# vobbilis/kubernetes-rca-system

Measured on AMD Instinct MI355X. Metric: pod·timesteps scored/s + end-to-end RCA top-k latency (ms), 1M-pod mesh, higher is better.
Workload: dtype f32 (f64 window sums, int64 fixed-point ranks)

## Files before the change

kubernetes-rca-system_amd/csrc/score.hip:

```cpp
#include "krca_common.h"

#pragma clang fp contract(off)

namespace {

constexpr double kVarEps = 1e-12;

__global__ __launch_bounds__(256) void usage_flags_kernel(const float2* __restrict__ usage, int64_t P,
                                                          uint8_t* __restrict__ flags) {
  const int64_t stride = (int64_t)gridDim.x * blockDim.x;
  for (int64_t p = (int64_t)blockIdx.x * blockDim.x + threadIdx.x; p < P; p += stride) {
    const float2 u = usage[p];
    flags[p] = (u.x > 80.f ? KRCA_F_CPU80 : 0u) | (u.x > 90.f ? KRCA_F_CPU90 : 0u) |
               (u.y > 80.f ? KRCA_F_MEM80 : 0u) | (u.y > 90.f ? KRCA_F_MEM90 : 0u);
  }
}

struct StepState {
  double s1, s2;
  int cnt;
  double al, bl;
};

__device__ __forceinline__ void step(StepState& st, float v, float old, double Wd, double epsB, double thr2,
                                     bool last) {
  const double vd = (double)v;
  const double od = (double)old;
  const double A = fma(Wd, vd, -st.s1);
  const double B = fma(Wd, st.s2, -(st.s1 * st.s1));
  st.cnt += (B > epsB) && (fma(A, A, -(thr2 * B)) > 0.0);
  if (last) {
    st.al = A;
    st.bl = B;
  }
  st.s1 = (st.s1 + vd) - od;
  st.s2 = fma(-od, od, fma(vd, vd, st.s2));
}

struct NoEpisodes {
  static constexpr bool kTrack = false;
  struct Args {};
  __device__ __forceinline__ explicit NoEpisodes(Args) {}
};

struct TimelineOut {
  int32_t* onset;
  int32_t* last;
  int32_t* count;
  float* peak;
  int8_t* lead;
  uint8_t* n_metrics;
};

template <class Ep>
__device__ __forceinline__ void step(StepState& st, float v, float old, double Wd, double epsB, double thr2,
                                     bool last, Ep& ep, int t) {
  if constexpr (!Ep::kTrack) {
    step(st, v, old, Wd, epsB, thr2, last);
  } else {
    const double vd = (double)v;
    const double od = (double)old;
    const double A = fma(Wd, vd, -st.s1);
    const double B = fma(Wd, st.s2, -(st.s1 * st.s1));
    const bool exceed = (B > epsB) && (fma(A, A, -(thr2 * B)) > 0.0);
    st.cnt += exceed;
    if (exceed) ep.hit(t, A, B);
    if (last) {
      st.al = A;
      st.bl = B;
    }
    st.s1 = (st.s1 + vd) - od;
    st.s2 = fma(-od, od, fma(vd, vd, st.s2));
  }
}

struct Episodes {
  static constexpr bool kTrack = true;
  struct Args {
    int gap, min_count;
    TimelineOut out;
  };
  int gap, min_count;
  int c_on, c_last, c_cnt;
  float c_peak;
  int k_on, k_last, k_cnt;
  float k_peak;
  __device__ __forceinline__ explicit Episodes(const Args& a)
      : gap(a.gap), min_count(a.min_count), c_on(-1), c_last(-1), c_cnt(0), c_peak(0.f), k_on(-1), k_last(-1),
        k_cnt(0), k_peak(-1.f) {}
  __device__ __forceinline__ void close() {
    if (c_cnt >= min_count && c_peak >= k_peak) {
      k_on = c_on;
      k_last = c_last;
      k_cnt = c_cnt;
      k_peak = c_peak;
    }
  }
  __device__ __forceinline__ void hit(int t, double A, double B) {
    const float z = (float)(fabs(A) / sqrt(B));
    if (c_cnt > 0 && t - c_last <= gap) {
      c_last = t;
      ++c_cnt;
      c_peak = fmaxf(c_peak, z);
    } else {
      close();
      c_on = c_last = t;
      c_cnt = 1;
      c_peak = z;
    }
  }
};

struct StreamEpisodes : Episodes {
  struct Args {
    int gap, min_count, H;
    int32_t* state;
    TimelineOut out;
  };
  int H;
  bool c_dirty, k_dirty;
  __device__ __forceinline__ explicit StreamEpisodes(const Args& a)
      : Episodes(Episodes::Args{a.gap, a.min_count, a.out}), H(a.H), c_dirty(false), k_dirty(false) {}
  __device__ __forceinline__ void load(const int32_t* p, int64_t S, int64_t sl) {
    c_on = p[sl];
    c_last = p[S + sl];
    c_cnt = p[2 * S + sl];
    c_peak = __builtin_bit_cast(float, p[3 * S + sl]);
    k_on = p[4 * S + sl];
    k_last = p[5 * S + sl];
    k_cnt = p[6 * S + sl];
    k_peak = __builtin_bit_cast(float, p[7 * S + sl]);
  }
  __device__ __forceinline__ void store(int32_t* p, int64_t S, int64_t sl) const {
    if (c_dirty) {
      p[sl] = c_on;
      p[S + sl] = c_last;
      p[2 * S + sl] = c_cnt;
      p[3 * S + sl] = __builtin_bit_cast(int32_t, c_peak);
    }
    if (k_dirty) {
      p[4 * S + sl] = k_on;
      p[5 * S + sl] = k_last;
      p[6 * S + sl] = k_cnt;
      p[7 * S + sl] = __builtin_bit_cast(int32_t, k_peak);
    }
  }
  __device__ __forceinline__ void close(int now) {
    if (c_cnt >= min_count && (k_cnt == 0 || now - k_last >= H || c_peak >= k_peak)) {
      k_on = c_on;
      k_last = c_last;
      k_cnt = c_cnt;
      k_peak = c_peak;
      k_dirty = true;
    }
  }
  __device__ __forceinline__ void hit(int t, double A, double B) {
    const float z = (float)(fabs(A) / sqrt(B));
    c_dirty = true;
    if (c_cnt > 0 && t - c_last <= gap) {
      c_last = t;
      ++c_cnt;
      c_peak = fmaxf(c_peak, z);
    } else {
      close(t);
      c_on = c_last = t;
      c_cnt = 1;
      c_peak = z;
    }
  }
};

__device__ __forceinline__ void timeline_combine(bool has, int e_on, int e_last, int e_cnt, float e_peak, int gap,
                                                 int64_t s, bool active, int M, const TimelineOut& o) {
  const int lane = threadIdx.x & 63;
  const int m = lane & (M - 1);
  float ap = has ? e_peak : -1.f;
  int am = m;
  for (int off = 1; off < M; off <<= 1) {
    const float op = __shfl_xor(ap, off, 64);
    const int om = __shfl_xor(am, off, 64);
    if (op > ap || (op == ap && om < am)) {
      ap = op;
      am = om;
    }
  }
  const int src = (lane & ~(M - 1)) + am;
  const int64_t a_on = __shfl(e_on, src, 64), a_last = __shfl(e_last, src, 64);
  const bool mem = has && (int64_t)e_on <= a_last + gap && a_on <= (int64_t)e_last + gap;
  long long first = mem ? (((long long)e_on << 8) | m) : INT64_MAX;
  int lastv = mem ? e_last : -1;
  int cnt = mem ? e_cnt : 0;
  int nm = mem ? 1 : 0;
  for (int off = 1; off < M; off <<= 1) {
    const long long of = __shfl_xor(first, off, 64);
    first = of < first ? of : first;
    const int ol = __shfl_xor(lastv, off, 64);
    lastv = ol > lastv ? ol : lastv;
    cnt += __shfl_xor(cnt, off, 64);
    nm += __shfl_xor(nm, off, 64);
  }
  if (!active || m != 0) return;
  const int64_t p = s / M;
  o.onset[p] = nm ? (int32_t)(first >> 8) : -1;
  o.last[p] = lastv;
  o.count[p] = cnt;
  o.peak[p] = nm ? ap : 0.f;
  o.lead[p] = nm ? (int8_t)(first & 0xff) : (int8_t)-1;
  o.n_metrics[p] = (uint8_t)nm;
}

__device__ __forceinline__ void timeline_epilogue(Episodes& ep, int64_t s, bool active, int M,
                                                  const TimelineOut& o) {
  ep.close();
  timeline_combine(active && ep.k_cnt > 0, ep.k_on, ep.k_last, ep.k_cnt, ep.k_peak, ep.gap, s, active, M, o);
}

__device__ __forceinline__ void stream_timeline_epilogue(const StreamEpisodes& ep, int now, int64_t s, bool active,
                                                         int M, const TimelineOut& o) {
  const bool k_ok = ep.k_cnt > 0 && now - ep.k_last < ep.H;
  const bool c_ok = ep.c_cnt >= ep.min_count && now - ep.c_last < ep.H;
  const bool use_c = c_ok && (!k_ok || ep.c_peak >= ep.k_peak);
  timeline_combine(active && (use_c || k_ok), use_c ? ep.c_on : ep.k_on, use_c ? ep.c_last : ep.k_last,
                   use_c ? ep.c_cnt : ep.k_cnt, use_c ? ep.c_peak : ep.k_peak, ep.gap, s, active, M, o);
}

__device__ __forceinline__ void pod_epilogue(const StepState& st, double epsB, int64_t s, bool active, int M, int T,
                                             const float* __restrict__ xs, int64_t S,
                                             float* __restrict__ z_last, float* __restrict__ score,
                                             int32_t* __restrict__ n_exceed, uint8_t* __restrict__ flags) {
  const bool has_z = st.bl > epsB;
  const float z = has_z ? (float)(st.al / sqrt(st.bl)) : 0.f;
  const int m = (int)(s & (M - 1));
  float vlast = (active && T > 0) ? xs[(int64_t)(T - 1) * S] : 0.f;
  unsigned f = 0;
  if (m == 0) f = (vlast > 80.f ? KRCA_F_CPU80 : 0u) | (vlast > 90.f ? KRCA_F_CPU90 : 0u);
  if (m == 1) f = (vlast > 80.f ? KRCA_F_MEM80 : 0u) | (vlast > 90.f ? KRCA_F_MEM90 : 0u);
  float az = fabsf(z);
  int cnt = st.cnt;
  for (int off = 1; off < M; off <<= 1) {
    az = fmaxf(az, __shfl_xor(az, off, 64));
    cnt += __shfl_xor(cnt, off, 64);
    f |= __shfl_xor(f, off, 64);
  }
  if (!active) return;
  z_last[s] = z;
  if (m == 0) {
    const int64_t p = s / M;
    score[p] = az;
    n_exceed[p] = cnt;
    flags[p] = (uint8_t)f;
  }
}

template <int W>
__global__ __launch_bounds__(256) void rolling_score_ring(const float* __restrict__ x, int64_t S, int T, int M,
                                                          double thr2, float* __restrict__ z_last,
                                                          float* __restrict__ score, int32_t* __restrict__ n_exceed,
                                                          uint8_t* __restrict__ flags) {
  const int64_t s = (int64_t)blockIdx.x * blockDim.x + threadIdx.x;
  const bool active = s < S;
  const float* xs = x + (active ? s : 0);
  const double Wd = (double)W, epsB = kVarEps * Wd * Wd;
  StepState st{0.0, 0.0, 0, 0.0, 0.0};
  float ring[W];
#pragma unroll
  for (int j = 0; j < W; ++j) {
    const float v = (j < T && active) ? xs[(int64_t)j * S] : 0.f;
    ring[j] = v;
    const double vd = (double)v;
    st.s1 = st.s1 + vd;
    st.s2 = fma(vd, vd, st.s2);
  }
  int t0 = W;
  for (; t0 + W <= T; t0 += W) {
    float nx[W];
#pragma unroll
    for (int j = 0; j < W; ++j) nx[j] = active ? xs[(int64_t)(t0 + j) * S] : 0.f;
#pragma unroll
    for (int j = 0; j < W; ++j) {
      step(st, nx[j], ring[j], Wd, epsB, thr2, t0 + j == T - 1);
      ring[j] = nx[j];
    }
  }
  if (t0 < T) {
#pragma unroll
    for (int j = 0; j < W; ++j) {
      if (t0 + j < T) {
        const float v = active ? xs[(int64_t)(t0 + j) * S] : 0.f;
        step(st, v, ring[j], Wd, epsB, thr2, t0 + j == T - 1);
        ring[j] = v;
      }
    }
  }
  pod_epilogue(st, epsB, s, active, M, T, xs, S, z_last, score, n_exceed, flags);
}

template <int AUX = 0>
__device__ __forceinline__ float bload(__amdgpu_buffer_rsrc_t r, uint32_t voff, uint32_t soff) {
  return __builtin_bit_cast(float, __builtin_amdgcn_raw_buffer_load_b32(r, (int)voff, (int)soff, AUX));
}

template <int C>
__device__ __forceinline__ __amdgpu_buffer_rsrc_t chunk_rsrc(const float* x, int64_t S, uint32_t rowb, int t,
                                                             int T) {
  int n = T - t;
  n = n < 0 ? 0 : (n > C ? C : n);
  n = __builtin_amdgcn_readfirstlane(n);
  return __builtin_amdgcn_make_buffer_rsrc((void*)(x + (int64_t)(n ? t : 0) * S), 0, (int)(rowb * (uint32_t)n),
                                           0x00020000);
}

struct SpanRows {
  const float* x;
  int64_t S;
  uint32_t rowb, voff;
  int T;
  __device__ __forceinline__ SpanRows(const float* x_, int64_t S_, int T_, int64_t s, bool active)
      : x(x_), S(S_), rowb((uint32_t)(S_ * 4)), voff(active ? (uint32_t)s * 4u : 0u), T(T_) {}
  template <int C, int AUX>
  __device__ __forceinline__ void load(int t, float (&out)[C]) const {
    const __amdgpu_buffer_rsrc_t rs = chunk_rsrc<C>(x, S, rowb, t, T);
#pragma unroll
    for (int j = 0; j < C; ++j) out[j] = bload<AUX>(rs, voff, rowb * j);
  }
};

struct BlockRows {
  const float* xb;
  int64_t S;
  uint32_t voff;
  int nrec;
  int T;
  __device__ __forceinline__ BlockRows(const float* x_, int64_t S_, int T_, int64_t, bool)
      : S(S_), voff(threadIdx.x * 4u), T(T_) {
    const int64_t s0 = (int64_t)blockIdx.x * blockDim.x;
    xb = x_ + s0;
    const int64_t n = S_ - s0;
    nrec = __builtin_amdgcn_readfirstlane((int)(4 * (n < (int64_t)blockDim.x ? n : (int64_t)blockDim.x)));
  }
  template <int C, int AUX>
  __device__ __forceinline__ void load(int t, float (&out)[C]) const {
#pragma unroll
    for (int j = 0; j < C; ++j) {
      const int tt = t + j;
      const bool in = tt < T;
      const __amdgpu_buffer_rsrc_t rs = __builtin_amdgcn_make_buffer_rsrc(
          (void*)(xb + (int64_t)(in ? tt : 0) * S), 0, in ? nrec : 0, 0x00020000);
      out[j] = bload<AUX>(rs, voff, 0);
    }
  }
};

template <int W, int C, int AUX = 0, class Rows = SpanRows, class Ep = NoEpisodes>
__global__ __launch_bounds__(256) void rolling_score_pipe(const float* __restrict__ x, int64_t S, int T, int M,
                                                          double thr2, float* __restrict__ z_last,
                                                          float* __restrict__ score, int32_t* __restrict__ n_exceed,
                                                          uint8_t* __restrict__ flags, typename Ep::Args targs) {
  static_assert(W % C == 0, "chunk must divide the window");
  constexpr int NC = W / C;
  const int64_t s = (int64_t)blockIdx.x * blockDim.x + threadIdx.x;
  const bool active = s < S;
  const Rows rows(x, S, T, s, active);
  const double Wd = (double)W, epsB = kVarEps * Wd * Wd;
  StepState st{0.0, 0.0, 0, 0.0, 0.0};
  Ep ep(targs);
  float ring[W];
  float cur[C];
#pragma unroll
  for (int c = 0; c < NC; ++c) {
    float tmp[C];
    rows.template load<C, AUX>(c * C, tmp);
#pragma unroll
    for (int j = 0; j < C; ++j) ring[c * C + j] = tmp[j];
  }
  rows.template load<C, AUX>(W, cur);
#pragma unroll
  for (int j = 0; j < W; ++j) {
    const double vd = (double)ring[j];
    st.s1 = st.s1 + vd;
    st.s2 = fma(vd, vd, st.s2);
  }
  int t0 = W;
  for (; t0 + W < T; t0 += W) {
#pragma unroll
    for (int c = 0; c < NC; ++c) {
      float nxt[C];
      rows.template load<C, AUX>(t0 + (c + 1) * C, nxt);
#pragma unroll
      for (int j = 0; j < C; ++j) {
        step(st, cur[j], ring[c * C + j], Wd, epsB, thr2, false, ep, t0 + c * C + j);
        ring[c * C + j] = cur[j];
      }
#pragma unroll
      for (int j = 0; j < C; ++j) cur[j] = nxt[j];
    }
  }
#pragma unroll
  for (int c = 0; c < NC; ++c) {
    if (c > 0) rows.template load<C, AUX>(t0 + c * C, cur);
#pragma unroll
    for (int j = 0; j < C; ++j) {
      const int t = t0 + c * C + j;
      if (t < T) {
        step(st, cur[j], ring[c * C + j], Wd, epsB, thr2, t == T - 1, ep, t);
        ring[c * C + j] = cur[j];
      }
    }
  }
  pod_epilogue(st, epsB, s, active, M, T, x + (active ? s : 0), S, z_last, score, n_exceed, flags);
  if constexpr (Ep::kTrack) timeline_epilogue(ep, s, active, M, targs.out);
}

template <class Ep = NoEpisodes>
__global__ __launch_bounds__(256) void rolling_score_reread(const float* __restrict__ x, int64_t S, int T, int W,
                                                            int M, double thr2, float* __restrict__ z_last,
                                                            float* __restrict__ score,
                                                            int32_t* __restrict__ n_exceed,
                                                            uint8_t* __restrict__ flags, typename Ep::Args targs) {
  const int64_t s = (int64_t)blockIdx.x * blockDim.x + threadIdx.x;
  const bool active = s < S;
  const float* xs = x + (active ? s : 0);
  const double Wd = (double)W, epsB = kVarEps * Wd * Wd;
  StepState st{0.0, 0.0, 0, 0.0, 0.0};
  Ep ep(targs);
  for (int j = 0; j < W && j < T; ++j) {
    const double vd = active ? (double)xs[(int64_t)j * S] : 0.0;
    st.s1 = st.s1 + vd;
    st.s2 = fma(vd, vd, st.s2);
  }
  for (int t = W; t < T; ++t) {
    const float v = active ? xs[(int64_t)t * S] : 0.f;
    const float o = active ? xs[(int64_t)(t - W) * S] : 0.f;
    step(st, v, o, Wd, epsB, thr2, t == T - 1, ep, t);
  }
  pod_epilogue(st, epsB, s, active, M, T, xs, S, z_last, score, n_exceed, flags);
  if constexpr (Ep::kTrack) timeline_epilogue(ep, s, active, M, targs.out);
}

struct StreamState {
  double* s1;
  double* s2;
  int32_t* cnt;
  float* ring;
  uint32_t* bits;
};

template <class Ep = NoEpisodes>
__global__ __launch_bounds__(256) void stream_score(const float* __restrict__ xn, int64_t S, int delta, int64_t t0,
                                                    int W, int H, int M, double thr2, StreamState stt,
                                                    float* __restrict__ z_last, float* __restrict__ score,
                                                    int32_t* __restrict__ n_exceed, uint8_t* __restrict__ flags,
                                                    typename Ep::Args targs) {
  const int64_t s = (int64_t)blockIdx.x * blockDim.x + threadIdx.x;
  const bool active = s < S;
  const int64_t sl = active ? s : 0;
  const double Wd = (double)W, epsB = kVarEps * Wd * Wd;
  StepState st{0.0, 0.0, 0, 0.0, 0.0};
  Ep ep(targs);
  int cnt = 0;
  if (t0 > 0) {
    st.s1 = stt.s1[sl];
    st.s2 = stt.s2[sl];
    cnt = stt.cnt[sl];
    if constexpr (Ep::kTrack) ep.load(targs.state, S, sl);
  } else if constexpr (Ep::kTrack) {
    ep.c_dirty = ep.k_dirty = true;
  }
  for (int j = 0; j < delta; ++j) {
    const int64_t t = t0 + j;
    const float v = xn[(int64_t)j * S + sl];
    float* rp = stt.ring + (t % W) * S + sl;
    if (t < W) {
      const double vd = (double)v;
      st.s1 = st.s1 + vd;
      st.s2 = fma(vd, vd, st.s2);
    } else {
      const float o = *rp;
      st.cnt = 0;
      step(st, v, o, Wd, epsB, thr2, j == delta - 1, ep, (int)t);
      const int64_t e = t - W;
      uint32_t* wp = stt.bits + ((e % H) >> 5) * S + sl;
      const uint32_t bit = 1u << ((e % H) & 31);
      const uint32_t word = *wp;
      cnt += st.cnt - ((word & bit) ? 1 : 0);
      if (active) *wp = st.cnt ? (word | bit) : (word & ~bit);
    }
    if (active) *rp = v;
  }
  if (active) {
    stt.s1[sl] = st.s1;
    stt.s2[sl] = st.s2;
    stt.cnt[sl] = cnt;
    if constexpr (Ep::kTrack) ep.store(targs.state, S, sl);
  }
  st.cnt = cnt;
  if (t0 + delta - 1 < W) st.bl = 0.0;
  pod_epilogue(st, epsB, s, active, M, delta, xn + sl, S, z_last, score, n_exceed, flags);
  if constexpr (Ep::kTrack) stream_timeline_epilogue(ep, (int)(t0 + delta - 1), s, active, M, targs.out);
}

constexpr int rows_per_chunk(int W) { return W == 60 ? 20 : (W == 30 ? 15 : (W == 20 ? 10 : W)); }
bool pipe_window(int W) { return W == 60 || W == 30 || W == 20 || W == 15 || W == 10; }

constexpr int kNt = 2;

struct ScoreCall {
  const float* x;
  int64_t S;
  int T, W, M;
  double thr2;
  float* z_last;
  float* score;
  int32_t* n_exceed;
  uint8_t* flags;
  dim3 grid;
  hipStream_t st;
};

template <class Ep>
void launch_reread(const ScoreCall& c, const typename Ep::Args& ea) {
  hipLaunchKernelGGL(rolling_score_reread<Ep>, c.grid, dim3(256), 0, c.st, c.x, c.S, c.T, c.W, c.M, c.thr2, c.z_last,
                     c.score, c.n_exceed, c.flags, ea);
}

template <int W, class Ep>
void launch_window(int variant, const ScoreCall& c, const typename Ep::Args& ea) {
  constexpr int C = rows_per_chunk(W);
  if (variant == KRCA_SCORE_PIPE)
    hipLaunchKernelGGL((rolling_score_pipe<W, C, kNt, SpanRows, Ep>), c.grid, dim3(256), 0, c.st, c.x, c.S, c.T, c.M,
                       c.thr2, c.z_last, c.score, c.n_exceed, c.flags, ea);
  else if (variant == KRCA_SCORE_PIPE_ROWS)
    hipLaunchKernelGGL((rolling_score_pipe<W, C, kNt, BlockRows, Ep>), c.grid, dim3(256), 0, c.st, c.x, c.S, c.T, c.M,
                       c.thr2, c.z_last, c.score, c.n_exceed, c.flags, ea);
  else if constexpr (Ep::kTrack)
    launch_reread<Ep>(c, ea);
  else
    hipLaunchKernelGGL(rolling_score_ring<W>, c.grid, dim3(256), 0, c.st, c.x, c.S, c.T, c.M, c.thr2, c.z_last, c.score,
                       c.n_exceed, c.flags);
}

template <class Ep>
int launch_score(const char* fn, const float* x, int64_t P, int32_t M, int32_t T, int32_t W, float z_thr, float* z_last,
                 float* score, int32_t* n_exceed, uint8_t* flags, const typename Ep::Args& ea, void* stream) {
  KRCA_CHECK_ARG(P >= 0 && T >= 0 && W >= 1, "%s: bad sizes P=%lld T=%d W=%d", fn, (long long)P, T, W);
  KRCA_CHECK_ARG(M >= 1 && M <= 64 && (M & (M - 1)) == 0, "%s: M=%d must be a power of two <= 64", fn, M);
  bool outs = x && z_last && score && n_exceed && flags;
  if constexpr (Ep::kTrack) {
    KRCA_CHECK_ARG(ea.gap >= 0 && ea.min_count >= 1, "%s: gap=%d must be >= 0, min_count=%d >= 1", fn, ea.gap,
                   ea.min_count);
    const TimelineOut& o = ea.out;
    outs = outs && o.onset && o.last && o.count && o.peak && o.lead && o.n_metrics;
  }
  if (P == 0) return KRCA_OK;
  KRCA_CHECK_ARG(outs, "%s: null pointer", fn);
  const int64_t S = P * (int64_t)M;
  KRCA_CHECK_ARG(S < (int64_t(1) << 32), "%s: P*M must be < 2^32", fn);
  const double thr2 = (double)z_thr * (double)z_thr;
  const dim3 grid((unsigned)krca::ceil_div(S, 256));
  const ScoreCall c{x, S, T, W, M, thr2, z_last, score, n_exceed, flags, grid, krca::as_stream(stream)};
  const int variant = krca_rolling_score_variant(P, M, T, W);
  switch (W) {
    case 60: launch_window<60, Ep>(variant, c, ea); break;
    case 30: launch_window<30, Ep>(variant, c, ea); break;
    case 20: launch_window<20, Ep>(variant, c, ea); break;
    case 15: launch_window<15, Ep>(variant, c, ea); break;
    case 10: launch_window<10, Ep>(variant, c, ea); break;
    default: launch_reread<Ep>(c, ea);
  }
  KRCA_LAUNCH_CHECK();
  return KRCA_OK;
}
}

extern "C" {

int64_t krca_stream_state_size(int64_t P, int32_t M, int32_t W, int32_t H) {
  const int64_t S = P * M;
  return S * (8 + 8 + 4) + (int64_t)W * S * 4 + krca::ceil_div(H, 32) * S * 4 + 64;
}

int64_t krca_stream_episode_state_size(int64_t P, int32_t M) { return P * (int64_t)M * 8 * 4; }

}

namespace {
template <class Ep>
int launch_stream(const char* fn, const float* x_new, int64_t P, int32_t M, int32_t delta, int64_t t0, int32_t W,
                  int32_t H, float z_thr, void* state, float* z_last, float* score, int32_t* n_exceed, uint8_t* flags,
                  const typename Ep::Args& ea, void* stream) {
  KRCA_CHECK_ARG(P >= 0 && delta >= 1 && t0 >= 0 && W >= 1 && H >= 1, "%s: bad sizes", fn);
  KRCA_CHECK_ARG(M >= 1 && M <= 64 && (M & (M - 1)) == 0, "%s: M=%d must be a power of two <= 64", fn, M);
  bool ptrs = x_new && state && z_last && score && n_exceed && flags;
  if constexpr (Ep::kTrack) {
    KRCA_CHECK_ARG(ea.gap >= 0 && ea.min_count >= 1, "%s: gap=%d must be >= 0, min_count=%d >= 1", fn, ea.gap,
                   ea.min_count);
    KRCA_CHECK_ARG(t0 + delta <= (int64_t)INT32_MAX, "%s: t0 + delta = %lld is past INT32_MAX (onsets are int32)", fn,
                   (long long)(t0 + delta));
    const TimelineOut& o = ea.out;
    ptrs = ptrs && ea.state && o.onset && o.last && o.count && o.peak && o.lead && o.n_metrics;
  }
  if (P == 0) return KRCA_OK;
  KRCA_CHECK_ARG(ptrs, "%s: null pointer", fn);
  if constexpr (Ep::kTrack)
    KRCA_CHECK_ARG(((uintptr_t)ea.state & 3) == 0, "%s: the episode state must be 4-byte aligned", fn);
  const int64_t S = P * (int64_t)M;
  char* b = reinterpret_cast<char*>(state);
  StreamState stt;
  stt.s1 = reinterpret_cast<double*>(b);
  stt.s2 = stt.s1 + S;
  stt.cnt = reinterpret_cast<int32_t*>(stt.s2 + S);
  stt.ring = reinterpret_cast<float*>(stt.cnt + S);
  stt.bits = reinterpret_cast<uint32_t*>(stt.ring + (int64_t)W * S);
  hipStream_t st = krca::as_stream(stream);
  if (t0 == 0) KRCA_HIP(hipMemsetAsync(stt.bits, 0, krca::ceil_div(H, 32) * S * 4, st));
  hipLaunchKernelGGL(stream_score<Ep>, dim3((unsigned)krca::ceil_div(S, 256)), dim3(256), 0, st, x_new, S, delta, t0, W,
                     H, M, (double)z_thr * (double)z_thr, stt, z_last, score, n_exceed, flags, ea);
  KRCA_LAUNCH_CHECK();
  return KRCA_OK;
}
}

extern "C" {

int krca_stream_score(const float* x_new, int64_t P, int32_t M, int32_t delta, int64_t t0, int32_t W, int32_t H,
                      float z_thr, void* state, float* z_last, float* score, int32_t* n_exceed, uint8_t* flags,
                      void* stream) {
  return launch_stream<NoEpisodes>("krca_stream_score", x_new, P, M, delta, t0, W, H, z_thr, state, z_last, score,
                                   n_exceed, flags, NoEpisodes::Args{}, stream);
}

int krca_stream_timeline(const float* x_new, int64_t P, int32_t M, int32_t delta, int64_t t0, int32_t W, int32_t H,
                         float z_thr, int32_t gap, int32_t min_count, void* state, void* ep_state, float* z_last,
                         float* score, int32_t* n_exceed, uint8_t* flags, int32_t* onset, int32_t* last, int32_t* count,
                         float* peak, int8_t* lead, uint8_t* n_metrics, void* stream) {
  const StreamEpisodes::Args ea{gap, min_count, H, reinterpret_cast<int32_t*>(ep_state),
                                TimelineOut{onset, last, count, peak, lead, n_metrics}};
  return launch_stream<StreamEpisodes>("krca_stream_timeline", x_new, P, M, delta, t0, W, H, z_thr, state, z_last,
                                       score, n_exceed, flags, ea, stream);
}

int krca_usage_flags(const float* usage, int64_t P, uint8_t* flags, void* stream) {
  KRCA_CHECK_ARG(P >= 0, "krca_usage_flags: P < 0");
  if (P == 0) return KRCA_OK;
  KRCA_CHECK_ARG(usage && flags, "krca_usage_flags: null pointer");
  const int64_t blocks = std::min<int64_t>(krca::ceil_div(P, 256), 4096);
  hipLaunchKernelGGL(usage_flags_kernel, dim3((unsigned)blocks), dim3(256), 0, krca::as_stream(stream),
                     reinterpret_cast<const float2*>(usage), P, flags);
  KRCA_LAUNCH_CHECK();
  return KRCA_OK;
}

int krca_rolling_score_variant(int64_t P, int32_t M, int32_t T, int32_t W) {
  const int impl = krca::tuning().score_impl;
  if (!pipe_window(W)) return KRCA_SCORE_REREAD;
  if (T <= W || impl == KRCA_SCORE_RING) return KRCA_SCORE_RING;
  if (impl == KRCA_SCORE_PIPE_ROWS) return KRCA_SCORE_PIPE_ROWS;
  return P * (int64_t)M * 4 * rows_per_chunk(W) < (int64_t(1) << 31) ? KRCA_SCORE_PIPE : KRCA_SCORE_PIPE_ROWS;
}

int krca_rolling_score(const float* x, int64_t P, int32_t M, int32_t T, int32_t W, float z_thr, float* z_last,
                       float* score, int32_t* n_exceed, uint8_t* flags, void* stream) {
  return launch_score<NoEpisodes>("krca_rolling_score", x, P, M, T, W, z_thr, z_last, score, n_exceed, flags,
                                  NoEpisodes::Args{}, stream);
}

int krca_rolling_timeline(const float* x, int64_t P, int32_t M, int32_t T, int32_t W, float z_thr, int32_t gap,
                          int32_t min_count, float* z_last, float* score, int32_t* n_exceed, uint8_t* flags,
                          int32_t* onset, int32_t* last, int32_t* count, float* peak, int8_t* lead,
                          uint8_t* n_metrics, void* stream) {
  const Episodes::Args tl{gap, min_count, TimelineOut{onset, last, count, peak, lead, n_metrics}};
  return launch_score<Episodes>("krca_rolling_timeline", x, P, M, T, W, z_thr, z_last, score, n_exceed, flags, tl,
                                stream);
}

}
```

Baseline: 192.9 billion.

## Replace chunked ring prefetch with a unified W+D slot ring walk

The rolling-score pipeline kernel moves into a shared header as score_walk, which keeps a ring of W+D slots. Each step's freed slot is immediately refilled with a row D steps ahead, instead of double-buffering a separate chunk. This removes the cur/nxt copy shuffle and lets loads overlap compute at a finer grain. Prefetch depths change slightly (W=20 now uses 10, W=15 uses 15, W=60 is configurable by macro). The larger fully unrolled ring raises register pressure, which could lower occupancy.

After: 201.3 billion (median of 6 runs). 1.04x the previous value.

```diff
diff --git a/kubernetes-rca-system_amd/csrc/score.hip b/kubernetes-rca-system_amd/csrc/score.hip
--- a/kubernetes-rca-system_amd/csrc/score.hip
+++ b/kubernetes-rca-system_amd/csrc/score.hip
@@ -1,10 +1,15 @@
 #include "krca_common.h"
+#include "score_walk.h"
 
 #pragma clang fp contract(off)
 
 namespace {
 
-constexpr double kVarEps = 1e-12;
+using krca_walk::kVarEps;
+using krca_walk::prefetch_rows;
+using krca_walk::score_walk;
+using krca_walk::step;
+using krca_walk::StepState;
 
 __global__ __launch_bounds__(256) void usage_flags_kernel(const float2* __restrict__ usage, int64_t P,
                                                           uint8_t* __restrict__ flags) {
@@ -16,27 +21,6 @@
   }
 }
 
-struct StepState {
-  double s1, s2;
-  int cnt;
-  double al, bl;
-};
-
-__device__ __forceinline__ void step(StepState& st, float v, float old, double Wd, double epsB, double thr2,
-                                     bool last) {
-  const double vd = (double)v;
-  const double od = (double)old;
-  const double A = fma(Wd, vd, -st.s1);
-  const double B = fma(Wd, st.s2, -(st.s1 * st.s1));
-  st.cnt += (B > epsB) && (fma(A, A, -(thr2 * B)) > 0.0);
-  if (last) {
-    st.al = A;
-    st.bl = B;
-  }
-  st.s1 = (st.s1 + vd) - od;
-  st.s2 = fma(-od, od, fma(vd, vd, st.s2));
-}
-
 struct NoEpisodes {
   static constexpr bool kTrack = false;
   struct Args {};
@@ -51,28 +35,6 @@
   int8_t* lead;
   uint8_t* n_metrics;
 };
-
-template <class Ep>
-__device__ __forceinline__ void step(StepState& st, float v, float old, double Wd, double epsB, double thr2,
-                                     bool last, Ep& ep, int t) {
-  if constexpr (!Ep::kTrack) {
-    step(st, v, old, Wd, epsB, thr2, last);
-  } else {
-    const double vd = (double)v;
-    const double od = (double)old;
-    const double A = fma(Wd, vd, -st.s1);
-    const double B = fma(Wd, st.s2, -(st.s1 * st.s1));
-    const bool exceed = (B > epsB) && (fma(A, A, -(thr2 * B)) > 0.0);
-    st.cnt += exceed;
-    if (exceed) ep.hit(t, A, B);
-    if (last) {
-      st.al = A;
-      st.bl = B;
-    }
-    st.s1 = (st.s1 + vd) - od;
-    st.s2 = fma(-od, od, fma(vd, vd, st.s2));
-  }
-}
 
 struct Episodes {
   static constexpr bool kTrack = true;
@@ -300,32 +262,36 @@
   return __builtin_bit_cast(float, __builtin_amdgcn_raw_buffer_load_b32(r, (int)voff, (int)soff, AUX));
 }
 
-template <int C>
-__device__ __forceinline__ __amdgpu_buffer_rsrc_t chunk_rsrc(const float* x, int64_t S, uint32_t rowb, int t,
-                                                             int T) {
-  int n = T - t;
-  n = n < 0 ? 0 : (n > C ? C : n);
-  n = __builtin_amdgcn_readfirstlane(n);
-  return __builtin_amdgcn_make_buffer_rsrc((void*)(x + (int64_t)(n ? t : 0) * S), 0, (int)(rowb * (uint32_t)n),
+__device__ __forceinline__ __amdgpu_buffer_rsrc_t span_rsrc(const float* x, int64_t S, uint32_t rowb, int t, int n,
+                                                            int T) {
+  int m = T - t;
+  m = m < 0 ? 0 : (m > n ? n : m);
+  m = __builtin_amdgcn_readfirstlane(m);
+  return __builtin_amdgcn_make_buffer_rsrc((void*)(x + (int64_t)(m ? t : 0) * S), 0, (int)(rowb * (uint32_t)m),
                                            0x00020000);
 }
 
 struct SpanRows {
+  struct Group {
+    __amdgpu_buffer_rsrc_t rs;
+  };
   const float* x;
   int64_t S;
   uint32_t rowb, voff;
   int T;
   __device__ __forceinline__ SpanRows(const float* x_, int64_t S_, int T_, int64_t s, bool active)
       : x(x_), S(S_), rowb((uint32_t)(S_ * 4)), voff(active ? (uint32_t)s * 4u : 0u), T(T_) {}
-  template <int C, int AUX>
-  __device__ __forceinline__ void load(int t, float (&out)[C]) const {
-    const __amdgpu_buffer_rsrc_t rs = chunk_rsrc<C>(x, S, rowb, t, T);
-#pragma unroll
-    for (int j = 0; j < C; ++j) out[j] = bload<AUX>(rs, voff, rowb * j);
+  __device__ __forceinline__ Group group(int t, int n) const { return Group{span_rsrc(x, S, rowb, t, n, T)}; }
+  template <int AUX>
+  __device__ __forceinline__ float load(const Group& g, int j) const {
+    return bload<AUX>(g.rs, voff, rowb * (uint32_t)j);
   }
 };
 
 struct BlockRows {
+  struct Group {
+    int t;
+  };
   const float* xb;
   int64_t S;
   uint32_t voff;
@@ -338,75 +304,29 @@
     const int64_t n = S_ - s0;
     nrec = __builtin_amdgcn_readfirstlane((int)(4 * (n < (int64_t)blockDim.x ? n : (int64_t)blockDim.x)));
   }
-  template <int C, int AUX>
-  __device__ __forceinline__ void load(int t, float (&out)[C]) const {
-#pragma unroll
-    for (int j = 0; j < C; ++j) {
-      const int tt = t + j;
-      const bool in = tt < T;
-      const __amdgpu_buffer_rsrc_t rs = __builtin_amdgcn_make_buffer_rsrc(
-          (void*)(xb + (int64_t)(in ? tt : 0) * S), 0, in ? nrec : 0, 0x00020000);
-      out[j] = bload<AUX>(rs, voff, 0);
-    }
-  }
-};
-
-template <int W, int C, int AUX = 0, class Rows = SpanRows, class Ep = NoEpisodes>
+  __device__ __forceinline__ Group group(int t, int) const { return Group{t}; }
+  template <int AUX>
+  __device__ __forceinline__ float load(const Group& g, int j) const {
+    const int tt = g.t + j;
+    const bool in = tt < T;
+    const __amdgpu_buffer_rsrc_t rs =
+        __builtin_amdgcn_make_buffer_rsrc((void*)(xb + (int64_t)(in ? tt : 0) * S), 0, in ? nrec : 0, 0x00020000);
+    return bload<AUX>(rs, voff, 0);
+  }
+};
+
+template <int W, int D, int AUX = 0, class Rows = SpanRows, class Ep = NoEpisodes>
 __global__ __launch_bounds__(256) void rolling_score_pipe(const float* __restrict__ x, int64_t S, int T, int M,
                                                           double thr2, float* __restrict__ z_last,
                                                           float* __restrict__ score, int32_t* __restrict__ n_exceed,
                                                           uint8_t* __restrict__ flags, typename Ep::Args targs) {
-  static_assert(W % C == 0, "chunk must divide the window");
-  constexpr int NC = W / C;
   const int64_t s = (int64_t)blockIdx.x * blockDim.x + threadIdx.x;
   const bool active = s < S;
   const Rows rows(x, S, T, s, active);
-  const double Wd = (double)W, epsB = kVarEps * Wd * Wd;
   StepState st{0.0, 0.0, 0, 0.0, 0.0};
   Ep ep(targs);
-  float ring[W];
-  float cur[C];
-#pragma unroll
-  for (int c = 0; c < NC; ++c) {
-    float tmp[C];
-    rows.template load<C, AUX>(c * C, tmp);
-#pragma unroll
-    for (int j = 0; j < C; ++j) ring[c * C + j] = tmp[j];
-  }
-  rows.template load<C, AUX>(W, cur);
-#pragma unroll
-  for (int j = 0; j < W; ++j) {
-    const double vd = (double)ring[j];
-    st.s1 = st.s1 + vd;
-    st.s2 = fma(vd, vd, st.s2);
-  }
-  int t0 = W;
-  for (; t0 + W < T; t0 += W) {
-#pragma unroll
-    for (int c = 0; c < NC; ++c) {
-      float nxt[C];
-      rows.template load<C, AUX>(t0 + (c + 1) * C, nxt);
-#pragma unroll
-      for (int j = 0; j < C; ++j) {
-        step(st, cur[j], ring[c * C + j], Wd, epsB, thr2, false, ep, t0 + c * C + j);
-        ring[c * C + j] = cur[j];
-      }
-#pragma unroll
-      for (int j = 0; j < C; ++j) cur[j] = nxt[j];
-    }
-  }
-#pragma unroll
-  for (int c = 0; c < NC; ++c) {
-    if (c > 0) rows.template load<C, AUX>(t0 + c * C, cur);
-#pragma unroll
-    for (int j = 0; j < C; ++j) {
-      const int t = t0 + c * C + j;
-      if (t < T) {
-        step(st, cur[j], ring[c * C + j], Wd, epsB, thr2, t == T - 1, ep, t);
-        ring[c * C + j] = cur[j];
-      }
-    }
-  }
+  score_walk<W, D, AUX>(rows, T, thr2, st, ep);
+  const double Wd = (double)W, epsB = kVarEps * Wd * Wd;
   pod_epilogue(st, epsB, s, active, M, T, x + (active ? s : 0), S, z_last, score, n_exceed, flags);
   if constexpr (Ep::kTrack) timeline_epilogue(ep, s, active, M, targs.out);
 }
@@ -499,7 +419,6 @@
   if constexpr (Ep::kTrack) stream_timeline_epilogue(ep, (int)(t0 + delta - 1), s, active, M, targs.out);
 }
 
-constexpr int rows_per_chunk(int W) { return W == 60 ? 20 : (W == 30 ? 15 : (W == 20 ? 10 : W)); }
 bool pipe_window(int W) { return W == 60 || W == 30 || W == 20 || W == 15 || W == 10; }
 
 constexpr int kNt = 2;
@@ -525,12 +444,12 @@
 
 template <int W, class Ep>
 void launch_window(int variant, const ScoreCall& c, const typename Ep::Args& ea) {
-  constexpr int C = rows_per_chunk(W);
+  constexpr int D = prefetch_rows(W);
   if (variant == KRCA_SCORE_PIPE)
-    hipLaunchKernelGGL((rolling_score_pipe<W, C, kNt, SpanRows, Ep>), c.grid, dim3(256), 0, c.st, c.x, c.S, c.T, c.M,
+    hipLaunchKernelGGL((rolling_score_pipe<W, D, kNt, SpanRows, Ep>), c.grid, dim3(256), 0, c.st, c.x, c.S, c.T, c.M,
                        c.thr2, c.z_last, c.score, c.n_exceed, c.flags, ea);
   else if (variant == KRCA_SCORE_PIPE_ROWS)
-    hipLaunchKernelGGL((rolling_score_pipe<W, C, kNt, BlockRows, Ep>), c.grid, dim3(256), 0, c.st, c.x, c.S, c.T, c.M,
+    hipLaunchKernelGGL((rolling_score_pipe<W, D, kNt, BlockRows, Ep>), c.grid, dim3(256), 0, c.st, c.x, c.S, c.T, c.M,
                        c.thr2, c.z_last, c.score, c.n_exceed, c.flags, ea);
   else if constexpr (Ep::kTrack)
     launch_reread<Ep>(c, ea);
@@ -655,7 +574,7 @@
   if (!pipe_window(W)) return KRCA_SCORE_REREAD;
   if (T <= W || impl == KRCA_SCORE_RING) return KRCA_SCORE_RING;
   if (impl == KRCA_SCORE_PIPE_ROWS) return KRCA_SCORE_PIPE_ROWS;
-  return P * (int64_t)M * 4 * rows_per_chunk(W) < (int64_t(1) << 31) ? KRCA_SCORE_PIPE : KRCA_SCORE_PIPE_ROWS;
+  return P * (int64_t)M * 4 * prefetch_rows(W) < (int64_t(1) << 31) ? KRCA_SCORE_PIPE : KRCA_SCORE_PIPE_ROWS;
 }
 
 int krca_rolling_score(const float* x, int64_t P, int32_t M, int32_t T, int32_t W, float z_thr, float* z_last,
diff --git a/kubernetes-rca-system_amd/csrc/score_walk.h b/kubernetes-rca-system_amd/csrc/score_walk.h
--- /dev/null
+++ b/kubernetes-rca-system_amd/csrc/score_walk.h
@@ -0,0 +1,110 @@
+#pragma once
+#include <cmath>
+#include <cstdint>
+
+#if defined(__HIPCC__)
+#define KRCA_WALK_FN __host__ __device__ __forceinline__
+#else
+#define KRCA_WALK_FN inline
+#endif
+
+#pragma clang fp contract(off)
+
+namespace krca_walk {
+
+constexpr double kVarEps = 1e-12;
+
+struct StepState {
+  double s1, s2;
+  int cnt;
+  double al, bl;
+};
+
+KRCA_WALK_FN void step(StepState& st, float v, float old, double Wd, double epsB, double thr2, bool last) {
+  const double vd = (double)v;
+  const double od = (double)old;
+  const double A = fma(Wd, vd, -st.s1);
+  const double B = fma(Wd, st.s2, -(st.s1 * st.s1));
+  st.cnt += (B > epsB) && (fma(A, A, -(thr2 * B)) > 0.0);
+  if (last) {
+    st.al = A;
+    st.bl = B;
+  }
+  st.s1 = (st.s1 + vd) - od;
+  st.s2 = fma(-od, od, fma(vd, vd, st.s2));
+}
+
+template <class Ep>
+KRCA_WALK_FN void step(StepState& st, float v, float old, double Wd, double epsB, double thr2, bool last, Ep& ep,
+                       int t) {
+  if constexpr (!Ep::kTrack) {
+    step(st, v, old, Wd, epsB, thr2, last);
+  } else {
+    const double vd = (double)v;
+    const double od = (double)old;
+    const double A = fma(Wd, vd, -st.s1);
+    const double B = fma(Wd, st.s2, -(st.s1 * st.s1));
+    const bool exceed = (B > epsB) && (fma(A, A, -(thr2 * B)) > 0.0);
+    st.cnt += exceed;
+    if (exceed) ep.hit(t, A, B);
+    if (last) {
+      st.al = A;
+      st.bl = B;
+    }
+    st.s1 = (st.s1 + vd) - od;
+    st.s2 = fma(-od, od, fma(vd, vd, st.s2));
+  }
+}
+
+#ifndef KRCA_SCORE_D60
+#define KRCA_SCORE_D60 20
+#endif
+constexpr int prefetch_rows(int W) { return W == 60 ? KRCA_SCORE_D60 : (W == 30 || W == 15 ? 15 : 10); }
+
+template <int W, int D, int AUX, class Rows, class Ep>
+KRCA_WALK_FN void score_walk(const Rows& rows, int T, double thr2, StepState& st, Ep& ep) {
+  constexpr int R = W + D;
+  const double Wd = (double)W, epsB = kVarEps * Wd * Wd;
+  float slot[R];
+#pragma unroll
+  for (int u0 = 0; u0 < R; u0 += D) {
+    const int n = R - u0 < D ? R - u0 : D;
+    const typename Rows::Group g = rows.group(u0, n);
+#pragma unroll
+    for (int j = 0; j < n; ++j) slot[u0 + j] = rows.template load<AUX>(g, j);
+  }
+#pragma unroll
+  for (int j = 0; j < W; ++j) {
+    const double vd = (double)slot[j];
+    st.s1 = st.s1 + vd;
+    st.s2 = fma(vd, vd, st.s2);
+  }
+  int tb = W;
+  for (; tb + R < T; tb += R) {
+#pragma unroll
+    for (int u0 = 0; u0 < R; u0 += D) {
+      const int n = R - u0 < D ? R - u0 : D;
+      const typename Rows::Group g = rows.group(tb + u0 + D, n);
+#pragma unroll
+      for (int j = 0; j < n; ++j) {
+        const int u = u0 + j;
+        step(st, slot[(W + u) % R], slot[u], Wd, epsB, thr2, false, ep, tb + u);
+        slot[u] = rows.template load<AUX>(g, j);
+      }
+    }
+  }
+#pragma unroll
+  for (int u0 = 0; u0 < R; u0 += D) {
+    const int n = R - u0 < D ? R - u0 : D;
+    const int nl = W - u0 < 0 ? 0 : (W - u0 < n ? W - u0 : n);
+    const typename Rows::Group g = rows.group(tb + u0 + D, nl);
+#pragma unroll
+    for (int j = 0; j < n; ++j) {
+      const int u = u0 + j, t = tb + u;
+      if (t < T) step(st, slot[(W + u) % R], slot[u], Wd, epsB, thr2, t == T - 1, ep, t);
+      if (j < nl) slot[u] = rows.template load<AUX>(g, j);
+    }
+  }
+}
+
+}
```
